# ZenHKD/ocr-vi-invoice

Measured on AMD Instinct MI355X. Metric: invoice images/sec end-to-end (det+rec), higher is better.
Workload: dtype f16x2

## Files before the change

### include/ocrvi.h

```cpp
#ifndef OCRVI_H
#define OCRVI_H

#include <stddef.h>
#include <stdint.h>

#ifdef __cplusplus
extern "C" {
#endif

#define OCRVI_OK 0
#define OCRVI_EINVAL (-1)
#define OCRVI_EHIP (-2)
#define OCRVI_ENOMEM (-3)
#define OCRVI_EBLOB (-4)
#define OCRVI_ERANGE (-5)

typedef enum { OCRVI_F32 = 0, OCRVI_BF16 = 1, OCRVI_F16 = 2, OCRVI_F16X2 = 3 } ocrvi_dtype;

const char* ocrvi_last_error(void);
int ocrvi_abi_version(void);

typedef struct ocrvi_det ocrvi_det;

typedef struct {
// ... 231 lines not shown
int ocrvi_test_conv(int device, int dtype, const float* x, const float* weight_host, const float* bias_host,
                    int N, int C, int H, int W, int Co, int ksize, int sh, int sw, int groups, int act, float* out,
                    int iters, float* avg_ms);
int ocrvi_test_conv_res(int device, int dtype, const float* x, const float* weight_host, const float* bias_host, const float* res, int N,
                        int C, int H, int W, int Co, int ksize, int res_mode, int act, float* out, int iters, float* avg_ms);
int ocrvi_test_bneck_tail(int device, const float* t1, const float* identity, const float* w2_host, const float* b2_host,
                          const float* w3_host, const float* b3_host, const float* w1_host, const float* b1_host, int N, int H, int W,
                          int no_phase_c, float* y_out, float* t1n_out, int iters, float* avg_ms);
int ocrvi_test_db_tail(int device, int dtype, const float* x, const float* dc1_w_bin_host, const float* dc1_b_bin_host,
                       const float* dc1_w_thr_host, const float* dc1_b_thr_host, const float* dc2_w_bin_host, const float* dc2_b_bin_host,
                       const float* dc2_w_thr_host, const float* dc2_b_thr_host, int N, int OH, int OW, int groups, int binary_only,
                       float* out, float* out2, int iters, float* avg_ms);
int ocrvi_test_gemm(int device, int dtype, const float* a, const float* weight_host, const float* bias_host, const float* res, int M,
                    int K, int N, int act, int res_post, int out_f32, float* out, int iters, float* avg_ms);
int ocrvi_test_gemm_raw(int device, int dtype, const float* a, const float* weight_host, const float* bias_host, const float* res, int M,
                        int K, int N, int act, int res_post, int out_f32, void* out_raw, float* out);
int ocrvi_test_ring_plan(int dtype, int amode, int M, int K, int N, int out_f32, int has_res, int n_cu, int32_t plan[8]);
int ocrvi_test_conv_raw(int device, int dtype, const float* x, const float* weight_host, const float* bias_host, const float* res, int N,
                        int C, int H, int W, int Co, int ksize, int sh, int sw, int groups, int act, int res_post, int out_f32, int in_place,
                        void* out_raw, float* out);
int ocrvi_test_gconv_plan(int dtype, int N, int C, int H, int W, int Co, int sh, int sw, int groups, int out_f32, int has_res, int n_cu,
                          int32_t plan[12]);
int ocrvi_test_stem_pool(int device, int dtype, const float* x, const float* weight_host, const float* bias_host, int N, int H, int W, int fused,
                         float* out, int iters, float* avg_ms);
int ocrvi_test_attention(int device, int dtype, const float* qkv, int B, int N, int heads, float* out, int iters,
                         float* avg_ms);

int ocrvi_test_mlp(int device, int dtype, float* x, const float* ln_g_host, const float* ln_b_host, const float* w1_host, const float* b1_host,
                   const float* w2_host, const float* b2_host, const float* next_g_host, const float* next_b_host, int want_xn, int M, int D,
                   float* xn_out, int iters, float* avg_ms);
int ocrvi_test_mlp_raw(int device, int dtype, float* x, const float* ln_g_host, const float* ln_b_host, const float* w1_host, const float* b1_host,
                       const float* w2_host, const float* b2_host, const float* next_g_host, const float* next_b_host, int M, int D, void* xn_raw,
                       float* xn_out, int iters, float* avg_ms);
int ocrvi_test_pack_f16x2(const float* src, size_t n, void* dst, float* wscale);

int ocrvi_test_layernorm(int device, int dtype, const float* x, int x_f32, int out_f32, const float* gamma_host, const float* beta_host,
                         int rows, int D, float* out);
int ocrvi_test_frm_vertical(int device, int dtype, const float* kv, const float* vq_host, int B, int H, int W, int D, float* out);
int ocrvi_test_asf(int device, int dtype, const float* p2, const float* p3, const float* p4, const float* p5, const float* w_host,
                   const float* b_host, int N, int H, int W, float* out);
int ocrvi_test_maxpool(int device, int dtype, const float* x, int N, int C, int H, int W, float* out);
int ocrvi_test_db_maps(int device, const float* bin_logits, const float* thresh_logits, float k, float* binary, float* thresh,
                       float* thresh_binary, size_t n);
int ocrvi_test_ctc_logsoftmax(int device, const float* logits, int ld, int B, int T, int C, float* log_probs, int32_t* argmax_ids);

int ocrvi_document_contour(const uint8_t* mask, int h, int w, int64_t stride, int32_t* quad , int32_t* found);
int ocrvi_document_contour_bits(const uint32_t* bits, int h, int w, int32_t* quad , int32_t* found);

#define OCRVI_DOC_AUTO 0
#define OCRVI_DOC_BRIGHT 1
#define OCRVI_DOC_DARK 2
int ocrvi_doc_working_size(int h, int w, int work_h, int32_t* ww, double* ratio);
int ocrvi_doc_mask_sizes(int n, int work_h, int ww_cap, size_t* workspace_bytes, size_t* mask_words);
int ocrvi_doc_mask_pages(int device, const int64_t* pages, int n, int work_h, int ww_cap, int polarity, uint32_t* masks, void* workspace,
                         size_t workspace_bytes, void* stream);
int ocrvi_doc_grey_u8(int device, const uint8_t* src, int h, int w, int work_h, uint8_t* dst, void* stream);
int ocrvi_doc_smooth_u8(int device, const uint8_t* src, int work_h, int ww, uint8_t* dst, void* stream);
int ocrvi_doc_histogram(int device, const uint8_t* src, int work_h, int ww, int32_t* hist, void* stream);
int ocrvi_doc_otsu(int device, const uint8_t* smooth, const int32_t* hist, int work_h, int ww, int polarity, int32_t* thr, void* stream);
int ocrvi_doc_mask_bits(int device, const uint8_t* smooth, int work_h, int ww, const int32_t* thr, uint32_t* bits, void* stream);

int ocrvi_prof_enable(int on);
int ocrvi_prof_reset(void);
int ocrvi_prof_report(char* buf, size_t cap);

#ifdef __cplusplus
// ... 4 lines not shown
```

### ocr_vi_invoice_amd/_lib.py

```python
from __future__ import annotations

import ctypes as C
import os
from typing import Optional

_HERE = os.path.dirname(os.path.abspath(__file__))
LIB_PATH = os.environ.get("OCRVI_LIB") or os.path.join(_HERE, "lib", "libocrvi.so")

OCRVI_F32, OCRVI_BF16, OCRVI_F16, OCRVI_F16X2 = 0, 1, 2, 3
DTYPES = {"f32": OCRVI_F32, "fp32": OCRVI_F32, "float32": OCRVI_F32, "bf16": OCRVI_BF16, "bfloat16": OCRVI_BF16,
          "f16": OCRVI_F16, "fp16": OCRVI_F16, "float16": OCRVI_F16,
          "f16x2": OCRVI_F16X2}
ABI_VERSION = 5

EXPORTS = [
    "ocrvi_last_error", "ocrvi_abi_version",
    "ocrvi_det_create", "ocrvi_det_destroy", "ocrvi_det_workspace_bytes", "ocrvi_det_forward", "ocrvi_det_debug_features",
    "ocrvi_rec_create", "ocrvi_rec_destroy", "ocrvi_rec_workspace_bytes", "ocrvi_rec_forward", "ocrvi_rec_debug_features",
    "ocrvi_ctc_greedy", "ocrvi_normalize_u8", "ocrvi_resize_u8", "ocrvi_crop_resize_normalize", "ocrvi_db_postprocess", "ocrvi_db_boxes_batch",
    "ocrvi_unclip_polygon", "ocrvi_db_components_workspace_bytes", "ocrvi_db_components", "ocrvi_db_boxes_batch_sparse",
    "ocrvi_test_deform_conv", "ocrvi_test_offset_conv", "ocrvi_test_conv", "ocrvi_test_gemm", "ocrvi_test_attention", "ocrvi_test_mlp", "ocrvi_test_stem_pool", "ocrvi_test_pack_f16x2",
    "ocrvi_prof_enable", "ocrvi_prof_reset", "ocrvi_prof_report",
    "ocrvi_det_status", "ocrvi_rec_status", "ocrvi_range_reset", "ocrvi_range_flag",
    "ocrvi_resize_normalize_pages", "ocrvi_crop_resize_normalize_pages", "ocrvi_db_boxes_pages",
    "ocrvi_det_binary_workspace_bytes", "ocrvi_det_forward_binary",
    "ocrvi_four_point_transform", "ocrvi_warp_perspective_u8", "ocrvi_warp_perspective_pages",
    "ocrvi_test_layernorm", "ocrvi_test_frm_vertical", "ocrvi_test_asf", "ocrvi_test_maxpool", "ocrvi_test_db_maps", "ocrvi_test_ctc_logsoftmax",
    "ocrvi_det_eval_workspace_bytes", "ocrvi_det_eval", "ocrvi_ctc_loss", "ocrvi_edit_distance",
    "ocrvi_test_deform_conv_res",
    "ocrvi_enhance_init", "ocrvi_enhance_tables", "ocrvi_enhance_workspace_bytes", "ocrvi_enhance_u8",
    "ocrvi_rgb_to_lab_u8", "ocrvi_lab_to_rgb_u8", "ocrvi_clahe_lab_u8", "ocrvi_nlm_lab_u8", "ocrvi_sharpen_u8",
    "ocrvi_min_area_quads", "ocrvi_quad_crops", "ocrvi_crop_quad_resize_normalize_pages", "ocrvi_crop_quad_resize_normalize",
    "ocrvi_jpeg_info", "ocrvi_jpeg_parse", "ocrvi_jpeg_table_entry", "ocrvi_jpeg_decode_pages",
    "ocrvi_test_conv_res", "ocrvi_test_db_tail",
    "ocrvi_db_target_jobs", "ocrvi_db_target_maps", "ocrvi_resize_normalize_pad_pages",
    "ocrvi_test_mlp_raw",
    "ocrvi_test_bneck_tail",
    "ocrvi_jpeg_quant_tables", "ocrvi_jpeg_encode_header", "ocrvi_jpeg_encode_sizes", "ocrvi_jpeg_encode_table_entry", "ocrvi_jpeg_encode_pages",
    "ocrvi_test_gemm_raw", "ocrvi_test_ring_plan",
    "ocrvi_overlay_segments", "ocrvi_overlay_pages",
    "ocrvi_test_deform_conv_raw", "ocrvi_test_dcn_plan",
    "ocrvi_test_conv_raw", "ocrvi_test_gconv_plan",
    "ocrvi_png_info", "ocrvi_png_parse", "ocrvi_png_table_entry", "ocrvi_png_plan", "ocrvi_png_decode_pages",
    "ocrvi_png_encode_sizes", "ocrvi_png_encode_table_entry", "ocrvi_png_encode_pages", "ocrvi_test_png_code_lengths",
    "ocrvi_document_contour", "ocrvi_document_contour_bits", "ocrvi_doc_working_size", "ocrvi_doc_mask_sizes", "ocrvi_doc_mask_pages",
    "ocrvi_doc_grey_u8", "ocrvi_doc_smooth_u8", "ocrvi_doc_histogram", "ocrvi_doc_otsu", "ocrvi_doc_mask_bits",
]
PAGE_ENTRY = 4
DET_EVAL_RECORD_BYTES = 104
DET_EVAL_INT_SLOTS = ("tp", "fp", "fn", "positive_count", "negatives", "negative_count")
DET_EVAL_F64_SLOTS = ("pos_bce", "topk_bce", "dice_inter", "pred_mask", "gt_mask", "l1_num", "thresh_mask")
CTC_LOSS_MAX_TARGET = 1024
EDIT_DISTANCE_MAX_LEN = 2048
CLAHE_WORKSPACE_BYTES = 16384
ENHANCE_MIN_SIDE = 16
DB_TARGET_GT, DB_TARGET_MASK, DB_TARGET_THRESH = 0, 1, 2
DB_TARGET_JOB = 8
DB_TARGET_MAX_SIDE = 16384
JPEG_ENTRY = 64
PNG_ENTRY = 16
JPEG_ENC_ENTRY = 64
JPEG_HEADER_MAX = 640
PNG_ENC_ENTRY = 16
PNG_ENC_BLOCK = 16384
OVERLAY_SEG = 8
OVERLAY_PRIM = 8
OVERLAY_MAX_COORD = 16384
DOC_POLARITIES = {"auto": 0, "bright": 1, "dark": 2}
DOC_WORK_H = 500
# ... 65 lines not shown
    lib.ocrvi_db_boxes_batch_sparse.argtypes = [vp, vp, vp, i32, vp, vp, C.c_longlong, i32, i32, i32, C.c_float, i32, C.c_float, C.c_float,
                                                C.c_double, C.c_double, i32, i32, i32, vp, vp, i32, vp, i32, vp]
    lib.ocrvi_unclip_polygon.argtypes = [vp, i32, C.c_double, vp, i32, C.POINTER(i32)]
    lib.ocrvi_db_boxes_batch.argtypes = [vp, i32, i32, i32, C.c_float, C.c_float, i32, C.c_float, C.c_float, C.c_double, C.c_double, i32, i32, i32,
                                         vp, vp, i32, vp, i32]
    lib.ocrvi_resize_normalize_pages.argtypes = [i32, vp, i32, i32, i32, f32p, vp]
    lib.ocrvi_crop_resize_normalize_pages.argtypes = [i32, vp, i32, i32p, i32, i32, i32, f32p, vp]
    lib.ocrvi_four_point_transform.argtypes = [vp, vp, vp, i32p, i32p]
    lib.ocrvi_warp_perspective_u8.argtypes = [i32, vp, i32, i32, vp, vp, i32, i32, vp]
    lib.ocrvi_warp_perspective_pages.argtypes = [i32, vp, vp, vp, i32, vp]
    lib.ocrvi_db_boxes_pages.argtypes = [vp, i32, i32, i32, C.c_float, C.c_float, i32, C.c_float, C.c_float, vp, vp, vp, vp, vp,
                                         vp, i32, vp, vp, vp, i32, vp, vp, i32]
    lib.ocrvi_test_deform_conv.argtypes = [i32, i32, f32p, f32p, f32p, vp, vp, i32, i32, i32, i32, i32, i32, i32, f32p, i32,
                                           C.POINTER(C.c_float)]
    lib.ocrvi_test_deform_conv_res.argtypes = [i32, i32, f32p, f32p, f32p, vp, vp, f32p, i32, i32, i32, i32, i32, i32, i32, f32p, i32,
                                               C.POINTER(C.c_float)]
    lib.ocrvi_test_offset_conv.argtypes = [i32, i32, f32p, vp, vp, i32, i32, i32, i32, i32, f32p, i32, C.POINTER(C.c_float)]
    lib.ocrvi_test_conv.argtypes = [i32, i32, f32p, vp, vp, i32, i32, i32, i32, i32, i32, i32, i32, i32, i32, f32p, i32,
                                    C.POINTER(C.c_float)]
    lib.ocrvi_test_conv_res.argtypes = [i32, i32, f32p, vp, vp, f32p, i32, i32, i32, i32, i32, i32, i32, i32, f32p, i32, C.POINTER(C.c_float)]
    lib.ocrvi_test_bneck_tail.argtypes = [i32, f32p, f32p, vp, vp, vp, vp, vp, vp, i32, i32, i32, i32, f32p, f32p, i32, C.POINTER(C.c_float)]
    lib.ocrvi_test_db_tail.argtypes = [i32, i32, f32p, vp, vp, vp, vp, vp, vp, vp, vp, i32, i32, i32, i32, i32, f32p, f32p, i32,
                                       C.POINTER(C.c_float)]
    lib.ocrvi_test_gemm.argtypes = [i32, i32, f32p, vp, vp, f32p, i32, i32, i32, i32, i32, i32, f32p, i32, C.POINTER(C.c_float)]
    lib.ocrvi_test_gemm_raw.argtypes = [i32, i32, f32p, vp, vp, f32p, i32, i32, i32, i32, i32, i32, vp, f32p]
    lib.ocrvi_test_ring_plan.argtypes = [i32, i32, i32, i32, i32, i32, i32, i32, C.POINTER(C.c_int32)]
    lib.ocrvi_test_deform_conv_raw.argtypes = [i32, i32, f32p, f32p, f32p, vp, vp, f32p, i32, i32, i32, i32, i32, i32, i32, vp, f32p]
    lib.ocrvi_test_dcn_plan.argtypes = [i32, i32, i32, i32, i32, i32, i32, i32, C.POINTER(C.c_int32)]
    lib.ocrvi_test_conv_raw.argtypes = [i32, i32, f32p, vp, vp, f32p] + [i32] * 13 + [vp, f32p]
    lib.ocrvi_test_gconv_plan.argtypes = [i32] * 12 + [C.POINTER(C.c_int32)]
    lib.ocrvi_test_stem_pool.argtypes = [i32, i32, f32p, vp, vp, i32, i32, i32, i32, f32p, i32, C.POINTER(C.c_float)]
    lib.ocrvi_test_attention.argtypes = [i32, i32, f32p, i32, i32, i32, f32p, i32, C.POINTER(C.c_float)]
    lib.ocrvi_test_mlp.argtypes = [i32, i32, f32p, vp, vp, vp, vp, vp, vp, vp, vp, i32, i32, i32, f32p, i32, C.POINTER(C.c_float)]
    lib.ocrvi_test_mlp_raw.argtypes = [i32, i32, f32p, vp, vp, vp, vp, vp, vp, vp, vp, i32, i32, vp, f32p, i32, C.POINTER(C.c_float)]
    lib.ocrvi_test_pack_f16x2.argtypes = [f32p, sz, vp, C.POINTER(C.c_float)]
    lib.ocrvi_test_layernorm.argtypes = [i32, i32, f32p, i32, i32, vp, vp, i32, i32, f32p]
    lib.ocrvi_test_frm_vertical.argtypes = [i32, i32, f32p, vp, i32, i32, i32, i32, f32p]
    lib.ocrvi_test_asf.argtypes = [i32, i32, f32p, f32p, f32p, f32p, vp, vp, i32, i32, i32, f32p]
    lib.ocrvi_test_maxpool.argtypes = [i32, i32, f32p, i32, i32, i32, i32, f32p]
    lib.ocrvi_test_db_maps.argtypes = [i32, f32p, f32p, C.c_float, f32p, f32p, f32p, sz]
    lib.ocrvi_test_ctc_logsoftmax.argtypes = [i32, f32p, i32, i32, i32, i32, f32p, i32p]
    lib.ocrvi_det_eval_workspace_bytes.argtypes = [i32, i32, i32, C.POINTER(sz)]
    lib.ocrvi_det_eval.argtypes = [i32, f32p, f32p, f32p, f32p, f32p, f32p, f32p, f32p, i32, i32, i32, C.c_double, vp, vp, sz, vp]
    lib.ocrvi_ctc_loss.argtypes = [i32, f32p, i32, i32, i32, i32p, i32, i32p, i32p, i32, vp, vp]
    lib.ocrvi_edit_distance.argtypes = [i32, i32p, i32, i32p, i32p, i32, i32p, i32, i32p, vp]
    lib.ocrvi_enhance_init.argtypes = [i32]
    lib.ocrvi_enhance_tables.argtypes = [vp, sz, C.POINTER(sz)]
    lib.ocrvi_enhance_workspace_bytes.argtypes = [i32, i32, C.POINTER(sz)]
    lib.ocrvi_enhance_u8.argtypes = [i32, vp, i32, i32, vp, vp, sz, vp]
    for name in ("ocrvi_rgb_to_lab_u8", "ocrvi_lab_to_rgb_u8", "ocrvi_nlm_lab_u8", "ocrvi_sharpen_u8"):
        getattr(lib, name).argtypes = [i32, vp, i32, i32, vp, vp]
    lib.ocrvi_clahe_lab_u8.argtypes = [i32, vp, i32, i32, vp, vp, sz, vp]
    lib.ocrvi_min_area_quads.argtypes = [vp, vp, i32, vp, vp]
    lib.ocrvi_quad_crops.argtypes = [vp, vp, i32, vp, vp, vp, vp]
    lib.ocrvi_crop_quad_resize_normalize_pages.argtypes = [i32, vp, i32, i32p, vp, i32, i32, i32, f32p, vp]
    lib.ocrvi_crop_quad_resize_normalize.argtypes = [i32, vp, i32, i32, i32, i32p, vp, i32, i32, i32, f32p, vp]
    lib.ocrvi_jpeg_info.argtypes = [vp, sz, C.POINTER(JpegInfo)]
    lib.ocrvi_jpeg_parse.argtypes = [vp, sz, vp, sz, C.POINTER(sz)]
    lib.ocrvi_jpeg_table_entry.argtypes = [C.POINTER(JpegInfo), sz, C.c_int64, C.c_int64, C.c_int64, C.c_int64, vp]
    lib.ocrvi_jpeg_decode_pages.argtypes = [i32, vp, vp, i32, vp, vp, sz, vp]
    lib.ocrvi_png_info.argtypes = [vp, sz, C.POINTER(PngInfo)]
    lib.ocrvi_png_parse.argtypes = [vp, sz, vp, sz, C.POINTER(sz)]
    lib.ocrvi_png_table_entry.argtypes = [C.POINTER(PngInfo), sz, C.c_int64, C.c_int64, C.c_int64, C.c_int64, vp]
    lib.ocrvi_png_plan.argtypes = [C.POINTER(PngInfo), C.POINTER(i32), C.POINTER(i32), C.POINTER(i32), C.POINTER(i32)]
    lib.ocrvi_png_decode_pages.argtypes = [i32, vp, vp, i32, vp, vp, sz, vp]
    lib.ocrvi_jpeg_quant_tables.argtypes = [i32, vp, vp]
# ... 78 lines not shown
```

### ocr_vi_invoice_amd/csrc/kernels.h

```cpp
#pragma once
#include "common.h"

namespace ocrvi {

int k_nchw3_to_nhwc4_pad(int dtype, const float* x, void* y, int N, int H, int W, int pad_t, int pad_l, int Hp, int Wp, hipStream_t s);
int k_maxpool3x3s2(int dtype, const void* x, void* y, int N, int H, int W, int C, hipStream_t s);
bool stem_pool_eligible(int dtype, int cout, int Kp, int KH, int H, int W);
int k_stem_pool(int dtype, const void* xpad, const void* w, const float* bias, float wscale, void* y, int N, int H, int W, int Hp, int Wp,
                hipStream_t s);
int k_layernorm(int dtype, const void* x, int x_f32, void* out, int out_f32, const float* gamma, const float* beta, int rows, int D,
                hipStream_t s);
bool mlp_fused_eligible(int dtype, int D);
bool mlp_x2_eligible(int dtype, int D);
void pack_mlp_x2_stream(const float* w1, const float* w2, int D, std::vector<char>& out);
int k_mlp_x2(float* x, void* xn, const float* ln_g, const float* ln_b, const float* next_g, const float* next_b, const void* wstream, const float* b1,
             const float* b2, int M, int D, hipStream_t s);
void pack_mlp_stream(const float* w1, const float* w2, int D, int dtype, std::vector<char>& out);
int k_mlp_fused(int dtype, float* x, void* xn, const float* ln_g, const float* ln_b, const float* next_g, const float* next_b, const void* wstream,
                const float* b1, const float* b2, int M, int D, hipStream_t s);
int k_cast_from_f32(int dtype, const float* x, void* y, size_t n, hipStream_t s);
int k_nhwc_to_nchw_f32(int dtype, const void* x, float* y, int N, int H, int W, int C, int ld, int coff, hipStream_t s);

int k_attention(int dtype, const void* qkv, void* out, int B, int N, int heads, hipStream_t s, void* scratch = nullptr);
size_t attention_scratch_bytes(int dtype, int B, int N, int heads);
int k_frm_vertical(int dtype, const void* kv, const float* vq, void* out, int B, int H, int W, int D, hipStream_t s);

int k_asf(int dtype, const void* p2, const void* p3, const void* p4, const void* p5, const float* w, const float* b, float* scratch, void* out,
          int N, int H, int W, hipStream_t s);
size_t asf_scratch_bytes(int N, int H, int W);
int k_db_maps(const float* bin_logits, const float* thresh_logits, float k, float* binary, float* thresh, float* thresh_binary, size_t n,
              hipStream_t s);

int k_ctc_logsoftmax_argmax(const float* logits, int ld, float* log_probs, int32_t* argmax_ids, int B, int T, int C, hipStream_t s);
int k_ctc_argmax_tbc(const float* log_probs, int32_t* argmax_ids, int B, int T, int C, hipStream_t s);
int k_ctc_collapse(const int32_t* argmax_ids, int32_t* ids, int32_t* lens, int B, int T, int blank, hipStream_t s);

}
```

### ocr_vi_invoice_amd/csrc/rec_model.hip

```cpp
#include <stdlib.h>
#include <string.h>

#include <algorithm>
#include <memory>

#include "model.h"

using namespace ocrvi;

namespace {
struct LNw { float *g = nullptr, *b = nullptr; };
struct MlpW {
    ConvLayer fc1, fc2;
    void* stream = nullptr;
    float *b1 = nullptr, *b2 = nullptr;
};
struct BlockW {
    bool local = false;
    LNw n1, n2;
    ConvLayer conv1, conv2;
    ConvLayer qkv, proj;
    MlpW mlp;
};
}

struct ocrvi_rec {
    int device = 0;
    ocrvi_rec_cfg cfg{};
    DeviceStore store;
    ConvLayer stem1, stem2;
    std::vector<BlockW> blocks[3];
    ConvLayer merge[2];
    LNw backbone_norm;
    LNw h_norm, h_norm2, v_norm_kv, v_norm2;
    ConvLayer h_qkv, h_proj, v_kv, v_proj, head;
    MlpW h_mlp, v_mlp;
    float* vq = nullptr;
    void *tap_bn = nullptr, *tap_frm = nullptr;
    RangeWatch range;
};

static int load_ln(DeviceStore& st, const Blob& b, const std::string& name, int d, LNw* ln) {
    OCRVI_TRY(load_vec(st, b, name + ".w", d, &ln->g));
    return load_vec(st, b, name + ".b", d, &ln->b);
}
static int load_lin(DeviceStore& st, const Blob& b, const std::string& name, int cout, int cin, int dt, ConvLayer* L, const float* extra = nullptr) {
    return load_conv(st, b, name, cout, cin, 0, 1, AM_CONV1, dt, true, L, extra);
}
static int load_mlp(DeviceStore& st, const Blob& b, const std::string& name, int d, int dt, MlpW* m) {
    OCRVI_TRY(load_lin(st, b, name + ".fc1", 4 * d, d, dt, &m->fc1));
    OCRVI_TRY(load_lin(st, b, name + ".fc2", d, 4 * d, dt, &m->fc2));
    static const bool fuse = !(getenv("OCRVI_MLP_FUSED") && atoi(getenv("OCRVI_MLP_FUSED")) == 0);
    if (fuse && mlp_fused_eligible(dt, d)) {
        const BlobTensor *w1 = nullptr, *b1 = nullptr, *w2 = nullptr, *b2 = nullptr;
        OCRVI_TRY(b.get(name + ".fc1.w", 4 * d, d, 0, 0, &w1));
        OCRVI_TRY(b.get(name + ".fc1.b", 4 * d, 0, 0, 0, &b1));
        OCRVI_TRY(b.get(name + ".fc2.w", d, 4 * d, 0, 0, &w2));
        OCRVI_TRY(b.get(name + ".fc2.b", d, 0, 0, 0, &b2));
        std::vector<char> packed;
        pack_mlp_stream(w1->data, w2->data, d, dt, packed);
        OCRVI_TRY(st.upload(packed.data(), packed.size(), &m->stream));
        OCRVI_TRY(st.upload(b1->data, (size_t)4 * d * 4, (void**)&m->b1));
        OCRVI_TRY(st.upload(b2->data, (size_t)d * 4, (void**)&m->b2));
    }
    return OCRVI_OK;
}

extern "C" int ocrvi_rec_create(int device, const void* blob_p, size_t blob_bytes, const ocrvi_rec_cfg* cfg, ocrvi_rec** out) {
    OCRVI_CHECK(cfg && out, OCRVI_EINVAL, "rec_create: null argument");
    OCRVI_CHECK(dtype_valid(cfg->dtype), OCRVI_EINVAL, "rec_create: bad dtype %d", cfg->dtype);
    for (int s = 0; s < 3; ++s)
        OCRVI_CHECK(cfg->dims[s] > 0 && cfg->dims[s] % 32 == 0 && cfg->num_blocks[s] > 0 && cfg->num_local[s] >= 0 &&
                        cfg->num_local[s] <= cfg->num_blocks[s],
                    OCRVI_EINVAL, "rec_create: bad stage %d config (dims must be multiples of 32)", s);
    OCRVI_CHECK(cfg->num_classes > 0 && cfg->num_classes % 4 == 0 && cfg->num_classes <= 1024, OCRVI_EINVAL,
                "rec_create: num_classes=%d must be a multiple of 4 and <= 1024", cfg->num_classes);
    DeviceGuard dg(device);
    OCRVI_HIP(dg.err);
    Blob blob;
    OCRVI_TRY(blob.parse(blob_p, blob_bytes));
    std::unique_ptr<ocrvi_rec> h(new ocrvi_rec);
    h->device = device;
    h->cfg = *cfg;
    const int dt = cfg->dtype;
    DeviceStore& st = h->store;
    const int d0 = cfg->dims[0], mid = d0 / 2;
    OCRVI_TRY(load_conv(st, blob, "stem.conv1", mid, 3, 3, 1, AM_ROWS, dt, true, &h->stem1));
    OCRVI_TRY(load_conv(st, blob, "stem.conv2", d0, mid, 3, 1, AM_CONV3, dt, true, &h->stem2));
    for (int s = 0; s < 3; ++s) {
        const int d = cfg->dims[s];
        h->blocks[s].resize(cfg->num_blocks[s]);
        for (int b = 0; b < cfg->num_blocks[s]; ++b) {
            BlockW& bw = h->blocks[s][b];
            const std::string p = "stages." + std::to_string(s) + ".blocks." + std::to_string(b);
            bw.local = b < cfg->num_local[s];
            OCRVI_TRY(load_ln(st, blob, p + ".norm1", d, &bw.n1));
            OCRVI_TRY(load_ln(st, blob, p + ".norm2", d, &bw.n2));
            if (bw.local) {
                const int groups = d / 32;
                OCRVI_TRY(load_conv(st, blob, p + ".mixer.conv1", d, 32, 3, groups, AM_CONV3, dt, true, &bw.conv1));
                OCRVI_TRY(load_conv(st, blob, p + ".mixer.conv2", d, 32, 3, groups, AM_CONV3, dt, true, &bw.conv2));
            } else {
                OCRVI_TRY(load_lin(st, blob, p + ".mixer.qkv", 3 * d, d, dt, &bw.qkv));
                OCRVI_TRY(load_lin(st, blob, p + ".mixer.proj", d, d, dt, &bw.proj));
            }
            OCRVI_TRY(load_mlp(st, blob, p + ".mlp", d, dt, &bw.mlp));
        }
        if (s < 2) OCRVI_TRY(load_conv(st, blob, "merges." + std::to_string(s), cfg->dims[s + 1], d, 3, 1, AM_CONV3, dt, true, &h->merge[s]));
    }
    const int d = cfg->dims[2];
    OCRVI_TRY(load_ln(st, blob, "backbone_norm", d, &h->backbone_norm));
    OCRVI_TRY(load_ln(st, blob, "frm.h_norm", d, &h->h_norm));
    OCRVI_TRY(load_ln(st, blob, "frm.h_norm2", d, &h->h_norm2));
    OCRVI_TRY(load_ln(st, blob, "frm.v_norm_kv", d, &h->v_norm_kv));
    OCRVI_TRY(load_ln(st, blob, "frm.v_norm2", d, &h->v_norm2));
    OCRVI_TRY(load_lin(st, blob, "frm.h_qkv", 3 * d, d, dt, &h->h_qkv));
    OCRVI_TRY(load_lin(st, blob, "frm.h_proj", d, d, dt, &h->h_proj));
    OCRVI_TRY(load_lin(st, blob, "frm.v_kv", 2 * d, d, dt, &h->v_kv));
    const BlobTensor* tok = nullptr;
    OCRVI_TRY(blob.get("frm.select_token", d, 0, 0, 0, &tok));
    OCRVI_TRY(load_lin(st, blob, "frm.v_proj", d, d, dt, &h->v_proj, tok->data));
    OCRVI_TRY(load_mlp(st, blob, "frm.h_mlp", d, dt, &h->h_mlp));
    OCRVI_TRY(load_mlp(st, blob, "frm.v_mlp", d, dt, &h->v_mlp));
    OCRVI_TRY(load_vec(st, blob, "frm.vq", d, &h->vq));
    OCRVI_TRY(load_lin(st, blob, "head", cfg->num_classes, d, dt, &h->head));
    OCRVI_TRY(finish_create(dt, h->range));
    *out = h.release();
    return OCRVI_OK;
}

extern "C" void ocrvi_rec_destroy(ocrvi_rec* h) {
    if (!h) return;
    DeviceGuard dg(h->device);
    delete h;
}

static int check_rec_shape(const ocrvi_rec* h, int B, int H, int W) {
    OCRVI_CHECK(h, OCRVI_EINVAL, "rec: null handle");
    OCRVI_CHECK(B > 0 && H > 0 && W > 0 && H % 16 == 0 && W % 4 == 0, OCRVI_EINVAL,
                "rec: input (B=%d,3,%d,%d) needs H %% 16 == 0 and W %% 4 == 0", B, H, W);
    const int tok = (H / 4) * (W / 4) / 2, tok_max = dtype_size(h->cfg.dtype) == 2 ? 1024 : 4096;
    OCRVI_CHECK(tok <= tok_max && H / 16 <= 8, OCRVI_EINVAL,
                "rec: %dx%d gives %d tokens in the first global-attention stage (at most %d in this mode) or more than 8 rows after the backbone", H, W, tok, tok_max);
    OCRVI_CHECK((size_t)B * (H / 2) * (W / 2) < ((size_t)1 << 23), OCRVI_EINVAL, "rec: batch of %d %dx%d crops too large for one call (chunk it)", B, H, W);
    return OCRVI_OK;
}

static int ln(Runner& r, const Tensor& x, const Tensor& y, const LNw& w) {
    if (r.dry()) return OCRVI_OK;
    return k_layernorm(r.dtype, x.p, x.f32, y.p, y.f32, w.g, w.b, (int)x.pixels(), x.c, r.stream);
}
static Tensor view(const Tensor& t, int n, int h, int w, int c) { return wrap(t.p, n, h, w, c, t.f32); }
static int attention(Runner& r, const Tensor& qkv, const Tensor& out, int seqs, int len, int heads) {
    const size_t mk = r.arena.mark(), sb = attention_scratch_bytes(r.dtype, seqs, len, heads);
    void* asc = sb ? r.arena.alloc(sb) : nullptr;
    if (!r.dry()) OCRVI_TRY(k_attention(r.dtype, qkv.p, out.p, seqs, len, heads, r.stream, asc));
    r.arena.release(mk);
    return OCRVI_OK;
}

static const LNw kCast{};
static int mlp_block(Runner& r, const Tensor& x, const Tensor& xn, const Tensor& hb, const LNw& n, const MlpW& m, int d, const LNw* next = nullptr,
                     bool* xn_done = nullptr) {
    const int rows = (int)x.pixels();
    if (xn_done) *xn_done = false;
    if (m.stream) {
        if (xn_done) *xn_done = next != nullptr;
        if (r.dry()) return OCRVI_OK;
        return k_mlp_fused(r.dtype, (float*)x.p, next ? xn.p : nullptr, n.g, n.b, next ? next->g : nullptr, next ? next->b : nullptr, m.stream, m.b1, m.b2,
                           rows, d, r.stream);
    }
    OCRVI_TRY(ln(r, x, xn, n));
    ConvOpts o1;
    o1.act = ACT_GELU;
    OCRVI_TRY(conv(r, m.fc1, view(xn, rows, 1, 1, d), view(hb, rows, 1, 1, 4 * d), o1));
    ConvOpts o2;
    o2.res = &x;
    o2.res_mode = RES_SAME;
    return conv(r, m.fc2, view(hb, rows, 1, 1, 4 * d), view(x, rows, 1, 1, d), o2);
}

static int rec_run(ocrvi_rec* h, Runner& r, const float* x, int B, int H, int W, float* log_probs, int32_t* argmax_ids, int32_t* ids,
                   int32_t* lens) {
    const ocrvi_rec_cfg& c = h->cfg;
    const int dt = c.dtype;
// ... 21 lines not shown
    Tensor logits = r.alloc(B * T, 1, 1, c.num_classes, true);
    int32_t* am_buf = (int32_t*)r.arena.alloc((size_t)B * T * 4);

    if (!r.dry()) OCRVI_TRY(k_nchw3_to_nhwc4_pad(dt, x, xpad.p, B, H, W, 1, 1, Hp, Wp, r.stream));
    {
        ConvOpts o;
        o.sh = o.sw = 2; o.pad = 1; o.act = ACT_GELU; o.Hp = Hp; o.Wp = Wp;
        OCRVI_TRY(conv(r, h->stem1, xpad, s1, o));
    }
    int cur = 0;
    Tensor xs = wrap(X[cur], B, Hs, Ws, c.dims[0], true);
    {
        ConvOpts o;
        o.sh = o.sw = 2; o.pad = 1; o.act = ACT_GELU;
        OCRVI_TRY(conv(r, h->stem2, s1, xs, o));
    }
    for (int s = 0; s < 3; ++s) {
        const int d = c.dims[s];
        const int rows = B * Hs * Ws;
        const Tensor xn = wrap(XN, B, Hs, Ws, d, false), t1 = wrap(T1, B, Hs, Ws, d, false), big = wrap(BIG, rows, 1, 1, 4 * d, false);
        bool xn_ready = false;
        const int nblk = (int)h->blocks[s].size();
        for (int bi = 0; bi < nblk; ++bi) {
            const BlockW& bw = h->blocks[s][bi];
            if (!xn_ready) OCRVI_TRY(ln(r, xs, xn, bw.n1));
            if (bw.local) {
                ConvOpts o;
                o.pad = 1; o.act = ACT_GELU;
                OCRVI_TRY(conv(r, bw.conv1, xn, t1, o));
                o.res = &xs; o.res_mode = RES_SAME; o.res_post = 1;
                OCRVI_TRY(conv(r, bw.conv2, t1, xs, o));
            } else {
                ConvOpts o;
                OCRVI_TRY(conv(r, bw.qkv, view(xn, rows, 1, 1, d), view(big, rows, 1, 1, 3 * d), o));
                OCRVI_TRY(attention(r, big, t1, B, Hs * Ws, d / 32));
                o.res = &xs; o.res_mode = RES_SAME;
                OCRVI_TRY(conv(r, bw.proj, view(t1, rows, 1, 1, d), view(xs, rows, 1, 1, d), o));
            }
            const LNw* next = bi + 1 < nblk ? &h->blocks[s][bi + 1].n1 : ((s < 2 && lowp) ? &kCast : nullptr);
            OCRVI_TRY(mlp_block(r, view(xs, rows, 1, 1, d), xn, big, bw.n2, bw.mlp, d, next, &xn_ready));
        }
        if (s < 2) {
            Tensor src = xn;
            if (lowp) {
                if (!xn_ready && !r.dry()) OCRVI_TRY(k_cast_from_f32(dt, (const float*)xs.p, xn.p, (size_t)rows * d, r.stream));
            } else {
                src = xs; src.f32 = false;
            }
            Tensor nx = wrap(X[cur ^ 1], B, Hs / 2, Ws, c.dims[s + 1], true);
            ConvOpts o;
            o.sh = 2; o.sw = 1; o.pad = 1;
            OCRVI_TRY(conv(r, h->merge[s], src, nx, o));
            xs = nx;
            cur ^= 1;
            Hs /= 2;
        }
    }
    const int rows = B * Hs * Ws;
    const Tensor bn = wrap(X[cur ^ 1], rows, 1, 1, d2, true);
    OCRVI_TRY(ln(r, view(xs, rows, 1, 1, d2), bn, h->backbone_norm));
    h->tap_bn = bn.p;
    const Tensor xr = wrap(X[cur], rows, 1, 1, d2, true);
    const Tensor xn = wrap(XN, rows, 1, 1, d2, false), t1 = wrap(T1, rows, 1, 1, d2, false), big = wrap(BIG, rows, 1, 1, 4 * d2, false);
    OCRVI_TRY(ln(r, bn, xn, h->h_norm));
    {
        ConvOpts o;
        OCRVI_TRY(conv(r, h->h_qkv, xn, view(big, rows, 1, 1, 3 * d2), o));
        OCRVI_TRY(attention(r, big, t1, B * Hs, Ws, d2 / 32));
        o.res = &bn; o.res_mode = RES_SAME;
        OCRVI_TRY(conv(r, h->h_proj, t1, xr, o));
    }
    bool xn_ready = false;
    OCRVI_TRY(mlp_block(r, xr, xn, big, h->h_norm2, h->h_mlp, d2, &h->v_norm_kv, &xn_ready));
    if (!xn_ready) OCRVI_TRY(ln(r, xr, xn, h->v_norm_kv));
    const int cols = B * Ws;
    const Tensor tq = wrap(r.arena.alloc((size_t)cols * d2 * 4), cols, 1, 1, d2, true);
    {
        ConvOpts o;
        OCRVI_TRY(conv(r, h->v_kv, xn, view(big, rows, 1, 1, 2 * d2), o));
        if (!r.dry()) OCRVI_TRY(k_frm_vertical(dt, big.p, h->vq, t1.p, B, Hs, Ws, d2, r.stream));
        OCRVI_TRY(conv(r, h->v_proj, view(t1, cols, 1, 1, d2), tq, o));
    }
    OCRVI_TRY(mlp_block(r, tq, view(xn, cols, 1, 1, d2), big, h->v_norm2, h->v_mlp, d2, lowp ? &kCast : nullptr, &xn_ready));
    h->tap_frm = tq.p;
    Tensor hin = view(xn, cols, 1, 1, d2);
    if (lowp) {
        if (!xn_ready && !r.dry()) OCRVI_TRY(k_cast_from_f32(dt, (const float*)tq.p, xn.p, (size_t)cols * d2, r.stream));
    } else {
        hin = tq; hin.f32 = false;
    }
    {
        ConvOpts o;
        OCRVI_TRY(conv(r, h->head, hin, logits, o));
    }
    if (!r.dry()) {
        int32_t* am = argmax_ids ? argmax_ids : am_buf;
        OCRVI_TRY(k_ctc_logsoftmax_argmax((const float*)logits.p, c.num_classes, log_probs, am, B, T, c.num_classes, r.stream));
        if (ids || lens) OCRVI_TRY(k_ctc_collapse(am, ids, lens, B, T, c.blank_id, r.stream));
    }
    return OCRVI_OK;
}

extern "C" int ocrvi_rec_workspace_bytes(const ocrvi_rec* h, int B, int H, int W, size_t* bytes) {
    return plan_workspace("rec_workspace_bytes", h, bytes, [&] { return check_rec_shape(h, B, H, W); }, [&](Runner& r) {
        return rec_run(const_cast<ocrvi_rec*>(h), r, nullptr, B, H, W, nullptr, nullptr, nullptr, nullptr);
    });
}

extern "C" int ocrvi_rec_forward(ocrvi_rec* h, const float* x, int B, int H, int W, float* log_probs, int32_t* argmax_ids, int32_t* ids,
                                 int32_t* lens, void* workspace, size_t workspace_bytes, void* stream) {
    return run_forward("rec_forward", h, x && workspace, "null input/workspace", workspace, workspace_bytes, stream,
                       [&] { return check_rec_shape(h, B, H, W); },
// ... 32 lines not shown
```

Measured before the change: 331.1.

## Add dedicated f16x2 linear kernel for recognizer QKV and KV projections

Adds a persistent f16x2 linear kernel that streams pre-packed, swizzled weight units through an LDS ring with async global-to-LDS loads. Activation rows stay resident in registers across all output units, and the bias is pre-scaled into shared memory. The kernel replaces the generic conv path for the attention QKV and FRM v_kv projections when K is 256 or 384. It is meant to cut the overhead and poor weight reuse of the general conv GEMM for these shapes, at the cost of a second packed weight copy and a new, complex code path.

```diff
diff --git a/include/ocrvi.h b/include/ocrvi.h
--- a/include/ocrvi.h
+++ b/include/ocrvi.h
@@ -287,6 +287,8 @@
 int ocrvi_test_mlp_raw(int device, int dtype, float* x, const float* ln_g_host, const float* ln_b_host, const float* w1_host, const float* b1_host,
                        const float* w2_host, const float* b2_host, const float* next_g_host, const float* next_b_host, int M, int D, void* xn_raw,
                        float* xn_out, int iters, float* avg_ms);
+int ocrvi_test_lin_x2(int device, const float* a, const float* weight_host, const float* bias_host, int M, int K, int N, int max_workgroups,
+                      void* out_raw, float* out, int iters, float* avg_ms);
 int ocrvi_test_pack_f16x2(const float* src, size_t n, void* dst, float* wscale);
 
 int ocrvi_test_layernorm(int device, int dtype, const float* x, int x_f32, int out_f32, const float* gamma_host, const float* beta_host,
diff --git a/ocr_vi_invoice_amd/_lib.py b/ocr_vi_invoice_amd/_lib.py
--- a/ocr_vi_invoice_amd/_lib.py
+++ b/ocr_vi_invoice_amd/_lib.py
@@ -34,7 +34,7 @@
     "ocrvi_jpeg_info", "ocrvi_jpeg_parse", "ocrvi_jpeg_table_entry", "ocrvi_jpeg_decode_pages",
     "ocrvi_test_conv_res", "ocrvi_test_db_tail",
     "ocrvi_db_target_jobs", "ocrvi_db_target_maps", "ocrvi_resize_normalize_pad_pages",
-    "ocrvi_test_mlp_raw",
+    "ocrvi_test_mlp_raw", "ocrvi_test_lin_x2",
     "ocrvi_test_bneck_tail",
     "ocrvi_jpeg_quant_tables", "ocrvi_jpeg_encode_header", "ocrvi_jpeg_encode_sizes", "ocrvi_jpeg_encode_table_entry", "ocrvi_jpeg_encode_pages",
     "ocrvi_test_gemm_raw", "ocrvi_test_ring_plan",
@@ -166,6 +166,7 @@
     lib.ocrvi_test_stem_pool.argtypes = [i32, i32, f32p, vp, vp, i32, i32, i32, i32, f32p, i32, C.POINTER(C.c_float)]
     lib.ocrvi_test_attention.argtypes = [i32, i32, f32p, i32, i32, i32, f32p, i32, C.POINTER(C.c_float)]
     lib.ocrvi_test_mlp.argtypes = [i32, i32, f32p, vp, vp, vp, vp, vp, vp, vp, vp, i32, i32, i32, f32p, i32, C.POINTER(C.c_float)]
+    lib.ocrvi_test_lin_x2.argtypes = [i32, f32p, vp, vp, i32, i32, i32, i32, vp, f32p, i32, C.POINTER(C.c_float)]
     lib.ocrvi_test_mlp_raw.argtypes = [i32, i32, f32p, vp, vp, vp, vp, vp, vp, vp, vp, i32, i32, vp, f32p, i32, C.POINTER(C.c_float)]
     lib.ocrvi_test_pack_f16x2.argtypes = [f32p, sz, vp, C.POINTER(C.c_float)]
     lib.ocrvi_test_layernorm.argtypes = [i32, i32, f32p, i32, i32, vp, vp, i32, i32, f32p]
diff --git a/ocr_vi_invoice_amd/csrc/kernels.h b/ocr_vi_invoice_amd/csrc/kernels.h
--- a/ocr_vi_invoice_amd/csrc/kernels.h
+++ b/ocr_vi_invoice_amd/csrc/kernels.h
@@ -16,6 +16,9 @@
 int k_mlp_x2(float* x, void* xn, const float* ln_g, const float* ln_b, const float* next_g, const float* next_b, const void* wstream, const float* b1,
              const float* b2, int M, int D, hipStream_t s);
 void pack_mlp_stream(const float* w1, const float* w2, int D, int dtype, std::vector<char>& out);
+bool lin_x2_eligible(int dtype, int K, int N);
+void pack_lin_x2_stream(const float* w, int N, int K, std::vector<char>& out);
+int k_lin_x2(const void* a, const void* wstream, const float* bias, void* out, int M, int K, int N, hipStream_t s, int max_workgroups = 0);
 int k_mlp_fused(int dtype, float* x, void* xn, const float* ln_g, const float* ln_b, const float* next_g, const float* next_b, const void* wstream,
                 const float* b1, const float* b2, int M, int D, hipStream_t s);
 int k_cast_from_f32(int dtype, const float* x, void* y, size_t n, hipStream_t s);
diff --git a/ocr_vi_invoice_amd/csrc/lin_x2.hip b/ocr_vi_invoice_amd/csrc/lin_x2.hip
--- /dev/null
+++ b/ocr_vi_invoice_amd/csrc/lin_x2.hip
@@ -0,0 +1,225 @@
+#include <stdlib.h>
+#include <string.h>
+
+#include "gemm_ring.h"
+#include "kernels.h"
+
+namespace ocrvi {
+OCRVI_RANGE_FLAG_TU()
+
+struct LinX2Params {
+    const char* a = nullptr;
+    const char* wstream = nullptr;
+    const float* bias = nullptr;
+    void* out = nullptr;
+    unsigned out_bytes = 0;
+    int M = 0, N = 0;
+};
+
+constexpr int LIN_X2_MAX_N = 2048;
+
+template <int K, int R>
+__global__ __launch_bounds__(512, 2) void lin_x2_kernel(const LinX2Params p) {
+    typedef f16x2_t T;
+    typedef Mma<T>::u4v U;
+    constexpr int NWV = 8, NT = 64 * NWV;
+    constexpr int KS = K / 32;
+    constexpr int UNIT = 32 * K * 4;
+    constexpr int IPW = UNIT / 1024 / NWV;
+    constexpr int PF = R - 1;
+    constexpr int NST = 2;
+    static_assert(UNIT % (1024 * NWV) == 0 && R >= 2 && (PF - 1) * IPW + NST < 64, "ring geometry");
+    extern __shared__ __attribute__((aligned(16))) char smem[];
+    const unsigned lds0 = (unsigned)(size_t)(__attribute__((address_space(3))) char*)smem;
+    float* const c_b = (float*)(smem + R * UNIT);
+
+    const int tid = threadIdx.x, lane = tid & 63;
+    const int wave = __builtin_amdgcn_readfirstlane(tid >> 6);
+    const int lr = lane & 15, g = lane >> 4;
+    const int q_tok = lane >> 2, q_g = lane & 3;
+    const int to_mfma = 4 * (4 * lr + g);
+    const int to_quad = 4 * (16 * q_g + q_tok);
+    const int NU = p.N >> 5;
+    const float ws = *(const float*)(p.wstream + (size_t)NU * UNIT);
+    {
+        const float bsc = 1.f / ws;
+        for (int i = tid; i < p.N; i += NT) c_b[i] = p.bias ? p.bias[i] * bsc : 0.f;
+    }
+    __syncthreads();
+
+    const int ntiles = (p.M + 127) >> 7;
+    const int G = gridDim.x;
+    const int my_tiles = (ntiles - (int)blockIdx.x + G - 1) / G;
+
+    const char* const wbase = uniform_ptr(p.wstream);
+    int prod_slot = 0, prod_mod = 0, cons_slot = 0;
+    auto issue_unit = [&]() {
+        const char* src = wbase + (size_t)prod_mod * UNIT + wave * 1024;
+        const unsigned dst = lds0 + prod_slot * UNIT + wave * 1024;
+#pragma unroll
+        for (int j = 0; j < IPW; ++j) glds16(src + j * (NWV * 1024), (unsigned)lane * 16u, __builtin_amdgcn_readfirstlane(dst + j * (NWV * 1024)));
+        prod_slot = prod_slot + 1 == R ? 0 : prod_slot + 1;
+        prod_mod = prod_mod + 1 == NU ? 0 : prod_mod + 1;
+    };
+    auto next_unit = [&]() -> const char* {
+        wait_vm_barrier<(PF - 1) * IPW + NST>();
+        issue_unit();
+        const char* s = smem + cons_slot * UNIT;
+        cons_slot = cons_slot + 1 == R ? 0 : cons_slot + 1;
+        return s;
+    };
+    for (int i = 0; i < PF; ++i) issue_unit();
+    const int sw = swz128(lr);
+    const int fo0 = ((2 * g) ^ sw) << 4, fo1 = ((2 * g + 1) ^ sw) << 4;
+    unsigned long long range_mask = 0;
+    const __amdgpu_buffer_rsrc_t orsrc = __builtin_amdgcn_make_buffer_rsrc(p.out, 0, (int)p.out_bytes, 0x00020000);
+    constexpr unsigned OOB = 0xfffffff0u;
+    const unsigned ldo_b = (unsigned)p.N * 4u;
+
+    for (int t = 0; t < my_tiles; ++t) {
+        const int tile = (int)blockIdx.x + t * G;
+        const int tok = tile * 128 + wave * 16 + q_tok;
+        U xH[KS], xL[KS];
+        {
+            const char* xr = p.a + (size_t)min(tok, p.M - 1) * (K * 4) + 32 * q_g;
+            uint4 c[KS][2];
+#pragma unroll
+            for (int ks = 0; ks < KS; ++ks) {
+                c[ks][0] = *(const uint4*)(xr + 128 * ks);
+                c[ks][1] = *(const uint4*)(xr + 128 * ks + 16);
+            }
+            auto mv = [&](unsigned v) { return (unsigned)__builtin_amdgcn_ds_bpermute(to_mfma, (int)v); };
+#pragma unroll
+            for (int ks = 0; ks < KS; ++ks) {
+                const uint4 c0 = make_uint4(mv(c[ks][0].x), mv(c[ks][0].y), mv(c[ks][0].z), mv(c[ks][0].w));
+                const uint4 c1 = make_uint4(mv(c[ks][1].x), mv(c[ks][1].y), mv(c[ks][1].z), mv(c[ks][1].w));
+                Mma<T>::regroup(c0, c1, xH[ks], xL[ks]);
+            }
+        }
+        wait_vm_only<0>();
+        const unsigned row_b = tok < p.M ? (unsigned)tok * ldo_b + 16u * (unsigned)q_g : OOB;
+
+        for (int u = 0; u < NU; ++u) {
+            const char* const U1 = next_unit();
+            f32x4 acc[2];
+            {
+                int l = threadIdx.x;
+                asm volatile("" : "+v"(l));
+                const float* bp = c_b + 32 * u + 4 * ((l & 63) >> 4);
+                const float4 b0 = *(const float4*)bp, b1 = *(const float4*)(bp + 16);
+                acc[0] = (f32x4){b0.x, b0.y, b0.z, b0.w};
+                acc[1] = (f32x4){b1.x, b1.y, b1.z, b1.w};
+            }
+            constexpr int P1 = 2;
+            uint4 wr[P1 + 1][2][2];
+            auto rd1 = [&](int ks, int set) {
+#pragma unroll
+                for (int a = 0; a < 2; ++a) {
+                    const char* r = U1 + (ks * 32 + 16 * a + lr) * 128;
+                    wr[set][a][0] = *(const uint4*)(r + fo0);
+                    wr[set][a][1] = *(const uint4*)(r + fo1);
+                }
+            };
+#pragma unroll
+            for (int i = 0; i < P1; ++i) rd1(i, i);
+            __builtin_amdgcn_sched_barrier(0);
+#pragma unroll
+            for (int ks = 0; ks < KS; ++ks) {
+                if (ks + P1 < KS) rd1(ks + P1, (ks + P1) % (P1 + 1));
+                __builtin_amdgcn_sched_barrier(0);
+#pragma unroll
+                for (int a = 0; a < 2; ++a)
+                    Mma<T>::three(Mma<T>::as_u4v(wr[ks % (P1 + 1)][a][0]), Mma<T>::as_u4v(wr[ks % (P1 + 1)][a][1]), xH[ks], xL[ks], acc[a]);
+                __builtin_amdgcn_sched_barrier(0);
+            }
+            const unsigned off = row_b != OOB ? row_b + 128u * (unsigned)u : OOB;
+#pragma unroll
+            for (int a = 0; a < 2; ++a) {
+                const float v[4] = {unscale<T>(acc[a][0], ws), unscale<T>(acc[a][1], ws), unscale<T>(acc[a][2], ws), unscale<T>(acc[a][3], ws)};
+                range_mask |= f16x2_out_of_range(v);
+                const uint4 e = Chunk<T>::pack(v);
+                auto mv = [&](unsigned x) { return (unsigned)__builtin_amdgcn_ds_bpermute(to_quad, (int)x); };
+                __builtin_amdgcn_raw_buffer_store_b128((u32x4){mv(e.x), mv(e.y), mv(e.z), mv(e.w)}, orsrc, off != OOB ? off + 64u * a : OOB, 0, 0);
+            }
+        }
+    }
+    wait_vm_only<0>();
+    f16x2_raise(range_mask);
+}
+
+bool lin_x2_eligible(int dtype, int K, int N) {
+    return mlp_x2_eligible(dtype, K) && (K == 256 || K == 384) && N > 0 && N % 32 == 0 && N <= LIN_X2_MAX_N;
+}
+
+void pack_lin_x2_stream(const float* w, int N, int K, std::vector<char>& out) {
+    const int KS = K / 32, NU = N / 32;
+    float scale = 1.f;
+    {
+        float mx = 0.f;
+        for (size_t i = 0; i < (size_t)N * K; ++i) mx = std::max(mx, fabsf(w[i]));
+        if (mx > 0.f && std::isfinite(mx)) {
+            int e = 0;
+            (void)frexpf(mx, &e);
+            scale = ldexpf(1.0f, std::min(std::max(14 - e, -100), 100));
+        }
+    }
+    const size_t nrows = (size_t)NU * KS * 32;
+    std::vector<float> buf(nrows * 32);
+    size_t o = 0;
+    for (int u = 0; u < NU; ++u)
+        for (int ks = 0; ks < KS; ++ks)
+            for (int row = 0; row < 32; ++row) {
+                const float* src = w + (size_t)(32 * u + row) * K + 32 * ks;
+                for (int e = 0; e < 32; ++e, ++o) buf[o] = src[e];
+            }
+    std::vector<char> chunks(buf.size() * 4);
+    convert_to_dtype(buf.data(), buf.size(), OCRVI_F16X2, chunks.data(), scale);
+    out.assign(chunks.size() + 4, 0);
+    for (size_t r = 0; r < nrows; ++r) {
+        const uint64_t* src = (const uint64_t*)(chunks.data() + r * 128);
+        uint64_t q[16];
+        for (int k = 0; k < 4; ++k) {
+            q[4 * k] = src[4 * k]; q[4 * k + 1] = src[4 * k + 2]; q[4 * k + 2] = src[4 * k + 1]; q[4 * k + 3] = src[4 * k + 3];
+        }
+        const int row = (int)(r & 31), sw = ((row >> 1) & 1) | (((row >> 3) & 1) << 2);
+        uint64_t* dst = (uint64_t*)(out.data() + r * 128);
+        for (int ch = 0; ch < 8; ++ch) {
+            dst[2 * (ch ^ sw)] = q[2 * ch];
+            dst[2 * (ch ^ sw) + 1] = q[2 * ch + 1];
+        }
+    }
+    const float tail = 1.0f / scale;
+    memcpy(out.data() + chunks.size(), &tail, 4);
+}
+
+template <int K, int R>
+static int launch_lin_x2(const LinX2Params& p, int max_workgroups, hipStream_t s) {
+    const int smem = R * 128 * K + LIN_X2_MAX_N * 4;
+    auto kern = lin_x2_kernel<K, R>;
+    OCRVI_TRY(ensure_max_smem((const void*)kern, smem));
+    int n_cu = 0;
+    OCRVI_TRY(device_cus(&n_cu));
+    const int ntiles = (p.M + 127) / 128;
+    int grid = std::min(ntiles, n_cu);
+    if (max_workgroups > 0) grid = std::min(grid, max_workgroups);
+    grid = cdiv(ntiles, cdiv(ntiles, grid));
+    hipLaunchKernelGGL(kern, dim3(grid), dim3(512), smem, s, p);
+    OCRVI_HIP(hipGetLastError());
+    return OCRVI_OK;
+}
+
+int k_lin_x2(const void* a, const void* wstream, const float* bias, void* out, int M, int K, int N, hipStream_t s, int max_workgroups) {
+    OCRVI_CHECK((K == 256 || K == 384) && N > 0 && N % 32 == 0 && N <= LIN_X2_MAX_N && a && wstream && out && M > 0 &&
+                    (size_t)M * N * 4 < ((size_t)1 << 32) - 16,
+                OCRVI_EINVAL, "lin_x2: bad argument (M %d, K %d, N %d)", M, K, N);
+    LinX2Params p;
+    p.a = (const char*)a; p.wstream = (const char*)wstream; p.bias = bias; p.out = out; p.M = M; p.N = N;
+    p.out_bytes = (unsigned)((size_t)M * N * 4);
+    char tag[64];
+    snprintf(tag, sizeof(tag), "lin_x2_k%d_f16x2", K);
+    ProfScope ps(tag, 2.0 * M * N * K, 4.0 * ((double)M * K + (double)N * K + (double)M * N), s);
+    if (K == 256) return launch_lin_x2<256, 4>(p, max_workgroups, s);
+    return launch_lin_x2<384, 3>(p, max_workgroups, s);
+}
+
+}
diff --git a/ocr_vi_invoice_amd/csrc/rec_model.hip b/ocr_vi_invoice_amd/csrc/rec_model.hip
--- a/ocr_vi_invoice_amd/csrc/rec_model.hip
+++ b/ocr_vi_invoice_amd/csrc/rec_model.hip
@@ -20,6 +20,7 @@
     LNw n1, n2;
     ConvLayer conv1, conv2;
     ConvLayer qkv, proj;
+    void* qkv_lin = nullptr;
     MlpW mlp;
 };
 }
@@ -34,6 +35,7 @@
     LNw backbone_norm;
     LNw h_norm, h_norm2, v_norm_kv, v_norm2;
     ConvLayer h_qkv, h_proj, v_kv, v_proj, head;
+    void *h_qkv_lin = nullptr, *v_kv_lin = nullptr;
     MlpW h_mlp, v_mlp;
     float* vq = nullptr;
     void *tap_bn = nullptr, *tap_frm = nullptr;
@@ -46,6 +48,15 @@
 }
 static int load_lin(DeviceStore& st, const Blob& b, const std::string& name, int cout, int cin, int dt, ConvLayer* L, const float* extra = nullptr) {
     return load_conv(st, b, name, cout, cin, 0, 1, AM_CONV1, dt, true, L, extra);
+}
+static int load_lin_x2(DeviceStore& st, const Blob& b, const std::string& name, int cout, int cin, int dt, ConvLayer* L, void** lin) {
+    OCRVI_TRY(load_lin(st, b, name, cout, cin, dt, L));
+    if (!lin_x2_eligible(dt, cin, cout)) return OCRVI_OK;
+    const BlobTensor* w = nullptr;
+    OCRVI_TRY(b.get(name + ".w", cout, cin, 0, 0, &w));
+    std::vector<char> packed;
+    pack_lin_x2_stream(w->data, cout, cin, packed);
+    return st.upload(packed.data(), packed.size(), lin);
 }
 static int load_mlp(DeviceStore& st, const Blob& b, const std::string& name, int d, int dt, MlpW* m) {
     OCRVI_TRY(load_lin(st, b, name + ".fc1", 4 * d, d, dt, &m->fc1));
@@ -101,7 +112,7 @@
                 OCRVI_TRY(load_conv(st, blob, p + ".mixer.conv1", d, 32, 3, groups, AM_CONV3, dt, true, &bw.conv1));
                 OCRVI_TRY(load_conv(st, blob, p + ".mixer.conv2", d, 32, 3, groups, AM_CONV3, dt, true, &bw.conv2));
             } else {
-                OCRVI_TRY(load_lin(st, blob, p + ".mixer.qkv", 3 * d, d, dt, &bw.qkv));
+                OCRVI_TRY(load_lin_x2(st, blob, p + ".mixer.qkv", 3 * d, d, dt, &bw.qkv, &bw.qkv_lin));
                 OCRVI_TRY(load_lin(st, blob, p + ".mixer.proj", d, d, dt, &bw.proj));
             }
             OCRVI_TRY(load_mlp(st, blob, p + ".mlp", d, dt, &bw.mlp));
@@ -114,9 +125,9 @@
     OCRVI_TRY(load_ln(st, blob, "frm.h_norm2", d, &h->h_norm2));
     OCRVI_TRY(load_ln(st, blob, "frm.v_norm_kv", d, &h->v_norm_kv));
     OCRVI_TRY(load_ln(st, blob, "frm.v_norm2", d, &h->v_norm2));
-    OCRVI_TRY(load_lin(st, blob, "frm.h_qkv", 3 * d, d, dt, &h->h_qkv));
+    OCRVI_TRY(load_lin_x2(st, blob, "frm.h_qkv", 3 * d, d, dt, &h->h_qkv, &h->h_qkv_lin));
     OCRVI_TRY(load_lin(st, blob, "frm.h_proj", d, d, dt, &h->h_proj));
-    OCRVI_TRY(load_lin(st, blob, "frm.v_kv", 2 * d, d, dt, &h->v_kv));
+    OCRVI_TRY(load_lin_x2(st, blob, "frm.v_kv", 2 * d, d, dt, &h->v_kv, &h->v_kv_lin));
     const BlobTensor* tok = nullptr;
     OCRVI_TRY(blob.get("frm.select_token", d, 0, 0, 0, &tok));
     OCRVI_TRY(load_lin(st, blob, "frm.v_proj", d, d, dt, &h->v_proj, tok->data));
@@ -151,6 +162,11 @@
     return k_layernorm(r.dtype, x.p, x.f32, y.p, y.f32, w.g, w.b, (int)x.pixels(), x.c, r.stream);
 }
 static Tensor view(const Tensor& t, int n, int h, int w, int c) { return wrap(t.p, n, h, w, c, t.f32); }
+static int linear(Runner& r, const ConvLayer& L, void* lin, const Tensor& x, const Tensor& y) {
+    if (!lin) return conv(r, L, x, y, ConvOpts());
+    if (r.dry()) return OCRVI_OK;
+    return k_lin_x2(x.p, lin, L.bias, y.p, (int)x.pixels(), x.c, y.c, r.stream);
+}
 static int attention(Runner& r, const Tensor& qkv, const Tensor& out, int seqs, int len, int heads) {
     const size_t mk = r.arena.mark(), sb = attention_scratch_bytes(r.dtype, seqs, len, heads);
     void* asc = sb ? r.arena.alloc(sb) : nullptr;
@@ -238,7 +254,7 @@
                 OCRVI_TRY(conv(r, bw.conv2, t1, xs, o));
             } else {
                 ConvOpts o;
-                OCRVI_TRY(conv(r, bw.qkv, view(xn, rows, 1, 1, d), view(big, rows, 1, 1, 3 * d), o));
+                OCRVI_TRY(linear(r, bw.qkv, bw.qkv_lin, view(xn, rows, 1, 1, d), view(big, rows, 1, 1, 3 * d)));
                 OCRVI_TRY(attention(r, big, t1, B, Hs * Ws, d / 32));
                 o.res = &xs; o.res_mode = RES_SAME;
                 OCRVI_TRY(conv(r, bw.proj, view(t1, rows, 1, 1, d), view(xs, rows, 1, 1, d), o));
@@ -271,7 +287,7 @@
     OCRVI_TRY(ln(r, bn, xn, h->h_norm));
     {
         ConvOpts o;
-        OCRVI_TRY(conv(r, h->h_qkv, xn, view(big, rows, 1, 1, 3 * d2), o));
+        OCRVI_TRY(linear(r, h->h_qkv, h->h_qkv_lin, xn, view(big, rows, 1, 1, 3 * d2)));
         OCRVI_TRY(attention(r, big, t1, B * Hs, Ws, d2 / 32));
         o.res = &bn; o.res_mode = RES_SAME;
         OCRVI_TRY(conv(r, h->h_proj, t1, xr, o));
@@ -283,7 +299,7 @@
     const Tensor tq = wrap(r.arena.alloc((size_t)cols * d2 * 4), cols, 1, 1, d2, true);
     {
         ConvOpts o;
-        OCRVI_TRY(conv(r, h->v_kv, xn, view(big, rows, 1, 1, 2 * d2), o));
+        OCRVI_TRY(linear(r, h->v_kv, h->v_kv_lin, xn, view(big, rows, 1, 1, 2 * d2)));
         if (!r.dry()) OCRVI_TRY(k_frm_vertical(dt, big.p, h->vq, t1.p, B, Hs, Ws, d2, r.stream));
         OCRVI_TRY(conv(r, h->v_proj, view(t1, cols, 1, 1, d2), tq, o));
     }
```

Result: faster. 335.2 (median of 6 runs) (+1.2%).
